# allenai/gpv-1

Hardware: AMD Instinct MI355X
Metric: images/sec/node (train step, 480x640, bs32/GPU) (higher is better)
Workload: dtype bf16; 1 GPU; GPV-1 (ResNet-50 + 6+6 DETR layers, 100 queries, RoI head, BERT-base, 3 co-attention, 3 text-decoder layers, V=10000) CocoCaptioning-only train step, dropout 0.1, AdamW; global_batch=32, image=480x640, parallelism=dp1

## Files before the change

### gpv-1_amd/csrc/misc.hip

```cpp
#include "common.h"
#include <cstdlib>
#include "../../include/gpv_hip.h"

namespace {

inline int64_t cdiv(int64_t a, int64_t b) { return (a + b - 1) / b; }
inline int grid1d(int64_t n, int per_block) {
  int64_t g = cdiv(n, per_block);
  return (int)(g > 8192 ? 8192 : (g < 1 ? 1 : g));
}

template <bool HALF> __device__ __forceinline__ float row_sum(float v) {
  if (HALF) {
#pragma unroll
    for (int o = 16; o > 0; o >>= 1) v += __shfl_xor(v, o);
    return v;
  }
  return wave_sum(v);
}

template <typename T, int NV, bool HALF>
__global__ __launch_bounds__(256) void ln_fwd_kernel(const T* __restrict__ x, const T* __restrict__ s,
                                                     const float* __restrict__ gamma, const float* __restrict__ beta,
                                                     T* __restrict__ y, float* __restrict__ mean, float* __restrict__ rstd,
// ... 339 lines not shown
}

template <typename T>
__global__ __launch_bounds__(256) void colsum8_kernel(const T* __restrict__ x, float* __restrict__ out, int rows, int cols, int64_t ld,
                                                      int ct, int rows_per_block) {
  const int cx = threadIdx.x % ct, ry = threadIdx.x / ct, rl = 256 / ct;
  const int c = ((int)blockIdx.x * ct + cx) * 8;
  if (c >= cols) return;
  const int r0 = blockIdx.y * rows_per_block, r1 = min(rows, r0 + rows_per_block);
  float s[8] = {0.f, 0.f, 0.f, 0.f, 0.f, 0.f, 0.f, 0.f};
  for (int r = r0 + ry; r < r1; r += rl) {
    float v[8];
    Ld8<T>::ld(x + (int64_t)r * ld + c, v);
#pragma unroll
    for (int e = 0; e < 8; ++e) s[e] += v[e];
  }
#pragma unroll
  for (int e = 0; e < 8; ++e) atomicAdd(&out[c + e], s[e]);
}

template <typename TS, typename TD>
__global__ void cast_kernel(const TS* __restrict__ s, TD* __restrict__ d, int64_t n) {
  for (int64_t i = blockIdx.x * (int64_t)blockDim.x + threadIdx.x; i < n; i += (int64_t)gridDim.x * blockDim.x) d[i] = (TD)(float)s[i];
}

template <typename TD>
__global__ __launch_bounds__(256) void cast_rowscale_t_kernel(const float* __restrict__ src, const float* __restrict__ scale,
                                                              TD* __restrict__ dst, TD* __restrict__ dstT, int rows, int cols) {
  __shared__ float tile[32][33];
  const int c0 = blockIdx.x * 32, r0 = blockIdx.y * 32;
  const int tx = threadIdx.x & 31, ty = threadIdx.x >> 5;
  for (int j = ty; j < 32; j += 8) {
    int r = r0 + j, c = c0 + tx;
    float v = 0.f;
    if (r < rows && c < cols) {
      v = src[(int64_t)r * cols + c] * (scale ? scale[r] : 1.f);
      if (dst) dst[(int64_t)r * cols + c] = (TD)v;
    }
    tile[j][tx] = v;
  }
  if (!dstT) return;
  __syncthreads();
  for (int j = ty; j < 32; j += 8) {
    int c = c0 + j, r = r0 + tx;
    if (r < rows && c < cols) dstT[(int64_t)c * rows + r] = (TD)tile[tx][j];
  }
}

struct TcGroup {
  int n;
  int tile_start[GPV_TC_GROUP_MAX + 1];
  gpv_tc_problem prob[GPV_TC_GROUP_MAX];
};
template <typename TD>
__global__ __launch_bounds__(256) void cast_transpose_group_kernel(const TcGroup g) {
  __shared__ float tile[64][65];
  int pi = 0;
  while (pi + 1 < g.n && (int)blockIdx.x >= g.tile_start[pi + 1]) ++pi;
  const gpv_tc_problem q = g.prob[pi];
  const int t = (int)blockIdx.x - g.tile_start[pi];
  const int tc = (q.cols + 63) >> 6;
  const int r0 = (t / tc) * 64, c0 = (t % tc) * 64;
  const int lr = threadIdx.x >> 2, seg = (threadIdx.x & 3) * 16;
  {
    const int r = r0 + lr, c = c0 + seg;
    const float* sp = q.src + (int64_t)r * q.cols + c;
    if (r < q.rows && c + 16 <= q.cols && (q.cols & 3) == 0) {
#pragma unroll
      for (int v = 0; v < 4; ++v) {
        const float4 x = *reinterpret_cast<const float4*>(sp + 4 * v);
        tile[lr][seg + 4 * v] = x.x; tile[lr][seg + 4 * v + 1] = x.y; tile[lr][seg + 4 * v + 2] = x.z; tile[lr][seg + 4 * v + 3] = x.w;
      }
    } else {
#pragma unroll
      for (int e = 0; e < 16; ++e) tile[lr][seg + e] = (r < q.rows && c + e < q.cols) ? sp[e] : 0.f;
    }
  }
  __syncthreads();
  {
    const int c = c0 + lr, r = r0 + seg;
    if (c >= q.cols) return;
    TD* dp = reinterpret_cast<TD*>(q.dstT) + (int64_t)c * q.rows + r;
    float v[16];
#pragma unroll
    for (int e = 0; e < 16; ++e) v[e] = tile[seg + e][lr];
    if (r + 16 <= q.rows && (q.rows & 7) == 0) {
      Ld8<TD>::st(dp, v);
      Ld8<TD>::st(dp + 8, v + 8);
    } else {
#pragma unroll
      for (int e = 0; e < 16; ++e)
        if (r + e < q.rows) dp[e] = (TD)v[e];
    }
  }
}

template <typename TD>
__global__ __launch_bounds__(256) void prep_conv_w_kernel(const float* __restrict__ src, const float* __restrict__ scale,
                                                          TD* __restrict__ wf, TD* __restrict__ wd, int Cout, int T, int Cin) {
  __shared__ float tile[32][33];
  const int t = blockIdx.z;
  const int ci0 = blockIdx.x * 32, co0 = blockIdx.y * 32;
  const int tx = threadIdx.x & 31, ty = threadIdx.x >> 5;
  for (int j = ty; j < 32; j += 8) {
    int co = co0 + j, ci = ci0 + tx;
    float v = 0.f;
    if (co < Cout && ci < Cin) {
      v = src[((int64_t)co * T + t) * Cin + ci] * (scale ? scale[co] : 1.f);
      if (wf) wf[((int64_t)co * T + t) * Cin + ci] = (TD)v;
    }
    tile[j][tx] = v;
  }
  if (!wd) return;
  __syncthreads();
  for (int j = ty; j < 32; j += 8) {
    int ci = ci0 + j, co = co0 + tx;
    if (co < Cout && ci < Cin) wd[((int64_t)ci * T + t) * Cout + co] = (TD)tile[tx][j];
  }
}

template <typename TT, typename TO>
__global__ void embedding_kernel(const TT* __restrict__ table, const int64_t* __restrict__ ids, TO* __restrict__ out, int64_t n_ids,
                                 int dim) {
  for (int64_t i = blockIdx.x * (int64_t)blockDim.x + threadIdx.x; i < n_ids * dim; i += (int64_t)gridDim.x * blockDim.x) {
    int64_t r = i / dim;
    int c = (int)(i - r * dim);
    out[i] = (TO)(float)table[ids[r] * dim + c];
  }
}

template <typename T>
__global__ void dropout_kernel(const T* __restrict__ x, T* __restrict__ y, int64_t n, uint32_t dthresh, float dscale, uint64_t seed,
                               const uint64_t* seed_dev) {
  seed = eff_seed(seed, seed_dev);
  for (int64_t i = blockIdx.x * (int64_t)blockDim.x + threadIdx.x; i < n; i += (int64_t)gridDim.x * blockDim.x)
    y[i] = (T)(drop_keep(seed, (uint64_t)i, dthresh) ? (float)x[i] * dscale : 0.f);
}

template <typename T>
// ... 340 lines not shown
extern "C" int gpv_colsum(const void* x, float* out, int rows, int cols, int64_t ld, int dtype, void* stream) {
  if (cols % 8 == 0 && ld % 8 == 0 && (reinterpret_cast<uintptr_t>(x) & 15) == 0) {
    const int c8 = cols / 8;
    int ct = 256;
    while (ct > 1 && ct / 2 >= c8) ct /= 2;
    const int gx = (c8 + ct - 1) / ct, rl = 256 / ct;
    int gy = (768 + gx - 1) / gx;
    if (gy > (rows + rl - 1) / rl) gy = (rows + rl - 1) / rl;
    if ((int64_t)gy * rl * cols > (1 << 17)) gy = (int)((1 << 17) / ((int64_t)rl * cols));
    if (gy < 1) gy = 1;
    const int rpb = (rows + gy - 1) / gy;
    dim3 grid(gx, (rows + rpb - 1) / rpb);
    if (dtype == GPV_BF16) hipLaunchKernelGGL((colsum8_kernel<bf16>), grid, dim3(256), 0, ST(stream), (const bf16*)x, out, rows, cols, ld, ct, rpb);
    else hipLaunchKernelGGL((colsum8_kernel<float>), grid, dim3(256), 0, ST(stream), (const float*)x, out, rows, cols, ld, ct, rpb);
    GPV_CHECK_LAUNCH();
    return 0;
  }
  int rpb = (rows + 255) / 256;
  if (rpb < 32) rpb = 32;
  dim3 grid((cols + 255) / 256, (rows + rpb - 1) / rpb);
  if (dtype == GPV_BF16) hipLaunchKernelGGL((colsum_kernel<bf16>), grid, dim3(256), 0, ST(stream), (const bf16*)x, out, rows, cols, ld, rpb);
  else hipLaunchKernelGGL((colsum_kernel<float>), grid, dim3(256), 0, ST(stream), (const float*)x, out, rows, cols, ld, rpb);
  GPV_CHECK_LAUNCH();
  return 0;
}

extern "C" int gpv_cast(const void* src, void* dst, int64_t n, int ds, int dd, void* stream) {
  dim3 g(grid1d(n, 256)), b(256);
  if (ds == GPV_F32 && dd == GPV_BF16) hipLaunchKernelGGL((cast_kernel<float, bf16>), g, b, 0, ST(stream), (const float*)src, (bf16*)dst, n);
  else if (ds == GPV_BF16 && dd == GPV_F32) hipLaunchKernelGGL((cast_kernel<bf16, float>), g, b, 0, ST(stream), (const bf16*)src, (float*)dst, n);
  else if (ds == GPV_F32 && dd == GPV_F32) hipLaunchKernelGGL((cast_kernel<float, float>), g, b, 0, ST(stream), (const float*)src, (float*)dst, n);
  else hipLaunchKernelGGL((cast_kernel<bf16, bf16>), g, b, 0, ST(stream), (const bf16*)src, (bf16*)dst, n);
  GPV_CHECK_LAUNCH();
  return 0;
}

extern "C" int gpv_cast_rowscale_t(const float* src, const float* scale, void* dst, void* dstT, int rows, int cols, int dtype_dst,
                                   void* stream) {
  dim3 grid((cols + 31) / 32, (rows + 31) / 32);
  if (dtype_dst == GPV_BF16) hipLaunchKernelGGL((cast_rowscale_t_kernel<bf16>), grid, dim3(256), 0, ST(stream), src, scale, (bf16*)dst, (bf16*)dstT, rows, cols);
  else hipLaunchKernelGGL((cast_rowscale_t_kernel<float>), grid, dim3(256), 0, ST(stream), src, scale, (float*)dst, (float*)dstT, rows, cols);
  GPV_CHECK_LAUNCH();
  return 0;
}

extern "C" int gpv_cast_transpose_group(const gpv_tc_problem* problems, int n, int dtype_dst, void* stream) {
  if (n < 0 || (n > 0 && !problems)) return (int)hipErrorInvalidValue;
  for (int i0 = 0; i0 < n; i0 += GPV_TC_GROUP_MAX) {
    TcGroup g;
    g.n = n - i0 < GPV_TC_GROUP_MAX ? n - i0 : GPV_TC_GROUP_MAX;
    int tiles = 0;
    for (int i = 0; i < g.n; ++i) {
      const gpv_tc_problem& q = problems[i0 + i];
      if (!q.src || !q.dstT || q.rows <= 0 || q.cols <= 0) return (int)hipErrorInvalidValue;
      g.prob[i] = q;
      g.tile_start[i] = tiles;
      tiles += ((q.rows + 63) / 64) * ((q.cols + 63) / 64);
    }
    g.tile_start[g.n] = tiles;
    if (dtype_dst == GPV_BF16) hipLaunchKernelGGL((cast_transpose_group_kernel<bf16>), dim3(tiles), dim3(256), 0, ST(stream), g);
    else hipLaunchKernelGGL((cast_transpose_group_kernel<float>), dim3(tiles), dim3(256), 0, ST(stream), g);
    GPV_CHECK_LAUNCH();
  }
  return 0;
}

extern "C" int gpv_prep_conv_weight(const float* src, const float* scale, void* wf, void* wd, int Cout, int T, int Cin, int dtype_dst,
                                    void* stream) {
  dim3 grid((Cin + 31) / 32, (Cout + 31) / 32, T);
  if (dtype_dst == GPV_BF16) hipLaunchKernelGGL((prep_conv_w_kernel<bf16>), grid, dim3(256), 0, ST(stream), src, scale, (bf16*)wf, (bf16*)wd, Cout, T, Cin);
  else hipLaunchKernelGGL((prep_conv_w_kernel<float>), grid, dim3(256), 0, ST(stream), src, scale, (float*)wf, (float*)wd, Cout, T, Cin);
  GPV_CHECK_LAUNCH();
  return 0;
}

extern "C" int gpv_embedding(const void* table, const int64_t* ids, void* out, int64_t n_ids, int dim, int dt, int dout, void* stream) {
  dim3 g(grid1d(n_ids * dim, 256)), b(256);
  if (dt == GPV_F32 && dout == GPV_BF16) hipLaunchKernelGGL((embedding_kernel<float, bf16>), g, b, 0, ST(stream), (const float*)table, ids, (bf16*)out, n_ids, dim);
  else if (dt == GPV_F32 && dout == GPV_F32) hipLaunchKernelGGL((embedding_kernel<float, float>), g, b, 0, ST(stream), (const float*)table, ids, (float*)out, n_ids, dim);
  else if (dt == GPV_BF16 && dout == GPV_BF16) hipLaunchKernelGGL((embedding_kernel<bf16, bf16>), g, b, 0, ST(stream), (const bf16*)table, ids, (bf16*)out, n_ids, dim);
  else return (int)hipErrorInvalidValue;
  GPV_CHECK_LAUNCH();
  return 0;
}

namespace gpvk { const uint64_t* g_seed_dev = nullptr; }
extern "C" int gpv_set_seed_device(const uint64_t* epoch) {
  gpvk::g_seed_dev = epoch;
  return 0;
}

extern "C" int gpv_dropout(const void* x, void* y, int64_t n, float p, uint64_t seed, int dtype, void* stream) {
  const uint32_t th = drop_thresh(p);
  const float sc = 1.f / (1.f - p);
  dim3 g(grid1d(n, 256)), b(256);
  if (dtype == GPV_BF16) hipLaunchKernelGGL((dropout_kernel<bf16>), g, b, 0, ST(stream), (const bf16*)x, (bf16*)y, n, th, sc, seed, gpvk::g_seed_dev);
  else hipLaunchKernelGGL((dropout_kernel<float>), g, b, 0, ST(stream), (const float*)x, (float*)y, n, th, sc, seed, gpvk::g_seed_dev);
  GPV_CHECK_LAUNCH();
  return 0;
}

extern "C" int gpv_relevance_condition(const void* x, const float* logits, const float* tokens, void* y, int rows, int dim, int dtype,
                                       void* stream) {
  dim3 g(grid1d((int64_t)rows * dim, 256)), b(256);
  if (dtype == GPV_BF16) hipLaunchKernelGGL((relevance_condition_kernel<bf16>), g, b, 0, ST(stream), (const bf16*)x, logits, tokens, (bf16*)y, rows, dim);
  else hipLaunchKernelGGL((relevance_condition_kernel<float>), g, b, 0, ST(stream), (const float*)x, logits, tokens, (float*)y, rows, dim);
  GPV_CHECK_LAUNCH();
  return 0;
}

extern "C" int gpv_act_fwd(const void* x, void* y, int64_t n, int act, int dtype, void* stream) {
  if (n % 8 || (act != GPV_ACT_RELU && act != GPV_ACT_GELU)) return (int)hipErrorInvalidValue;
// ... 52 lines not shown
```

### gpv-1_amd/hip.py

```python
import ctypes as C
import os
import threading

import torch

BF16, F32 = 0, 1
ACT_NONE, ACT_RELU, ACT_GELU = 0, 1, 2
KMAJOR, TRANS = 0, 1

_LIB = None
TUNING = os.environ.get('GPV_TUNING_LIB', '0') == '1'
_LIB_PATH = os.environ.get('GPV_HIP_LIB') or os.path.join(os.path.dirname(os.path.abspath(__file__)), 'csrc',
                                                          'libgpv_hip_tuning.so' if TUNING else 'libgpv_hip.so')


class GemmArgs(C.Structure):
    _fields_ = [('A', C.c_void_p), ('B', C.c_void_p), ('C', C.c_void_p),
                ('M', C.c_int), ('N', C.c_int), ('K', C.c_int), ('batch', C.c_int),
                ('lda', C.c_int64), ('ldb', C.c_int64), ('ldc', C.c_int64),
                ('sA', C.c_int64), ('sB', C.c_int64), ('sC', C.c_int64),
                ('layoutA', C.c_int), ('layoutB', C.c_int), ('dtype_in', C.c_int), ('dtype_out', C.c_int),
                ('alpha', C.c_float), ('rowscale', C.c_void_p), ('bias', C.c_void_p),
                ('res', C.c_void_p), ('ldr', C.c_int64), ('sR', C.c_int64),
                ('relu_mask', C.c_void_p), ('ldm', C.c_int64),
# ... 490 lines not shown
    return True


def ffn_fused_fwd(x, w1, b1, w2, b2, gamma, beta, h, y, out, mean, rstd, M, D, F, eps, drop_p=0.0, seed1=0, seed2=0, pos=None, out2=None):
    if not hasattr(lib(), 'gpv_ffn_fused_fwd'):
        return False
    ts = [t for t in (x, w1, w2, h, y, out, pos, out2) if t is not None]
    if not all(t.dtype == torch.bfloat16 and t.is_contiguous() for t in ts) or b1 is None or b2 is None:
        return False
    err = lib().gpv_ffn_fused_fwd(_p(x), _p(w1), _p(_f32(b1)), _p(w2), _p(_f32(b2)), _p(_f32(gamma)), _p(_f32(beta)), _p(h), _p(y), _p(out),
                                  _p(mean), _p(rstd), C.c_int(M), C.c_int(D), C.c_int(F), C.c_float(eps), C.c_float(drop_p), C.c_uint64(seed1), C.c_uint64(seed2),
                                  _p(pos), C.c_int(0 if pos is None else pos.numel() // D), _p(out2), _stream())
    if err == 801:
        return False
    _chk(err, 'gpv_ffn_fused_fwd')
    return True


def stem_pool(x, w, shift, y, B, Hp, Wp, CH, CW, PH, PW):
    if x.dtype != torch.bfloat16 or w.dtype != torch.bfloat16 or y.dtype != torch.bfloat16:
        raise TypeError('stem_pool: bf16 only')
    _chk(lib().gpv_stem_pool(_p(x), _p(w), _p(_f32(shift)), _p(y), B, Hp, Wp, CH, CW, PH, PW, _stream()), 'gpv_stem_pool')


def roi_weights(boxes, wgt, n_roi, H, W, ldw):
    _chk(lib().gpv_roi_weights(_p(_f32(boxes)), _p(wgt), n_roi, H, W, C.c_int64(ldw), dcode(wgt), _stream()),
         'gpv_roi_weights')


def add(a, b, y, n):
    _chk(lib().gpv_add(_p(a), _p(b), _p(y), C.c_int64(n), dcode(a), _stream()), 'gpv_add')


def add_rowbcast(a, b, y, rows_total, rows_b, cols):
    _chk(lib().gpv_add_rowbcast(_p(a), _p(b), _p(y), C.c_int64(rows_total), C.c_int64(rows_b), cols, dcode(a),
                                _stream()), 'gpv_add_rowbcast')


def colsum(x, out, rows, cols, ld):
    _chk(lib().gpv_colsum(_p(x), _p(_f32(out)), rows, cols, C.c_int64(ld), dcode(x), _stream()), 'gpv_colsum')


def cast(src, dst, n):
    _chk(lib().gpv_cast(_p(src), _p(dst), C.c_int64(n), dcode(src), dcode(dst), _stream()), 'gpv_cast')


def cast_rowscale_t(src, scale, dst, dstT, rows, cols):
    d = dst if dst is not None else dstT
    _chk(lib().gpv_cast_rowscale_t(_p(_f32(src)), _p(scale), _p(dst), _p(dstT), rows, cols, dcode(d), _stream()),
         'gpv_cast_rowscale_t')


class TCProblem(C.Structure):
    _fields_ = [('src', C.c_void_p), ('dstT', C.c_void_p), ('rows', C.c_int), ('cols', C.c_int)]


def cast_transpose_group(items):
    if not items:
        return
    arr = (TCProblem * len(items))()
    for t, (src, dstT) in zip(arr, items):
        _f32(src)
        rows, cols = src.shape
        assert src.is_contiguous() and dstT.is_contiguous() and tuple(dstT.shape) == (cols, rows)
        t.src, t.dstT, t.rows, t.cols = src.data_ptr(), dstT.data_ptr(), rows, cols
    _chk(lib().gpv_cast_transpose_group(arr, C.c_int(len(items)), C.c_int(dcode(items[0][1])), _stream()), 'gpv_cast_transpose_group')


def prep_conv_weight(src, scale, wf, wd, Cout, T, Cin):
    d = wf if wf is not None else wd
    _chk(lib().gpv_prep_conv_weight(_p(_f32(src)), _p(scale), _p(wf), _p(wd), Cout, T, Cin, dcode(d), _stream()),
         'gpv_prep_conv_weight')


def embedding(table, ids, out, n_ids, dim):
    _chk(lib().gpv_embedding(_p(table), _p(ids), _p(out), C.c_int64(n_ids), dim, dcode(table), dcode(out),
                             _stream()), 'gpv_embedding')


def dropout(x, y, n, p, seed):
    _chk(lib().gpv_dropout(_p(x), _p(y), C.c_int64(n), C.c_float(p), C.c_uint64(seed), dcode(x), _stream()),
         'gpv_dropout')


def relevance_condition(x, logits, tokens, y, rows, dim):
    _chk(lib().gpv_relevance_condition(_p(x), _p(_f32(logits)), _p(_f32(tokens)), _p(y), rows, dim, dcode(x),
                                       _stream()), 'gpv_relevance_condition')


def adamw(p, g, m, v, p_lowp, n, lr, beta1, beta2, eps, wd, bc1, bc2, gscale=None, seg_id=None, seg_live=None):
    _chk(lib().gpv_adamw(_p(p), _p(g), _p(m), _p(v), _p(p_lowp), C.c_int64(n), C.c_float(lr), C.c_float(beta1),
                         C.c_float(beta2), C.c_float(eps), C.c_float(wd), C.c_float(bc1), C.c_float(bc2),
                         _p(gscale), _p(seg_id), _p(seg_live), _stream()), 'gpv_adamw')


CLIP_PARTIALS = 1024


def clip_scale(g, max_norm, partial, gscale, pstep=None, live=None):
    n = 0 if g is None else g.numel()
    if g is not None and (not g.is_contiguous() or partial.numel() < CLIP_PARTIALS):
        raise ValueError('clip_scale: contiguous gradient range and >= CLIP_PARTIALS floats of scratch')
    for t in (pstep, live):
        if t is not None and t.dtype != torch.int32:
            raise TypeError('clip_scale: int32 step counts / liveness flags')
    _chk(lib().gpv_clip_scale(_p(_f32(g)), C.c_int64(n), C.c_float(max_norm), _p(_f32(partial)), _p(_f32(gscale)), _p(pstep), _p(live),
                              C.c_int(0 if pstep is None else pstep.numel()), _stream()), 'gpv_clip_scale')


def sumsq(x, n, out):
    _chk(lib().gpv_sumsq(_p(x), C.c_int64(n), _p(out), _stream()), 'gpv_sumsq')


def act_fwd(x, y, n, act):
    _chk(lib().gpv_act_fwd(_p(x), _p(y), C.c_int64(n), act, dcode(x), _stream()), 'gpv_act_fwd')


def argmax_rows(x, addend, out0=None, out1=None, table=None, pos_row=None, xnext=None):
    rows, V = x.shape
# ... 80 lines not shown
```

### gpv-1_amd/ops.py

```python
import math

import os
import weakref

import torch
from torch.autograd import Function

from . import hip

ACT_NONE, ACT_RELU, ACT_GELU = hip.ACT_NONE, hip.ACT_RELU, hip.ACT_GELU


class Runtime:
    def __init__(self):
        self.dtype = torch.bfloat16
        self.weights_epoch = 0
        self.static_epoch = 0
        self.seed = 0x5EED
        self.seed_explicit = False
        self._ctr = 0
        self.cache = {}
        self.backward_milestone = None
        self.split = None
        self.seed_dev = None
# ... 90 lines not shown

def _lp(p):
    N = p.shape[0]
    K = p.numel() // N
    if RT.dtype == torch.float32:
        src = p.detach().reshape(N, K)
        return src if src.is_contiguous() else src.contiguous()
    lp = getattr(p, '_gpv_lp', None)
    if lp is not None:
        if p._gpv_lp_static != RT.static_epoch:
            hip.cast(p._gpv_flat, lp, lp.numel())
            p._gpv_lp_static = RT.static_epoch
        return lp.view(N, K)
    key = ('lin', id(p), RT.dtype)
    hit = RT.cache.get(key)
    ep = RT.epoch_of(p)
    if hit is not None and hit[0] == ep:
        return hit[1]
    src = p.detach().reshape(N, K)
    if not src.is_contiguous():
        src = src.contiguous()
    w = torch.empty(N, K, device=p.device, dtype=RT.dtype)
    hip.cast(src, w, N * K)
    RT.cache[key] = (ep, w)
    return w


_T_PARAMS = {}
DX_MIRROR = os.environ.get('GPV_DX_MIRROR', '1') != '0'


def _lpT(p):
    N = p.shape[0]
    K = p.numel() // N
    key = ('linT', id(p), RT.dtype)
    hit = RT.cache.get(key)
    ep = RT.epoch_of(p)
    if hit is not None and hit[2]() is not p:
        hit = None
    if hit is not None and hit[0] == ep:
        return hit[1]
    src = getattr(p, '_gpv_flat', None)
    src = p.detach().reshape(N, K) if src is None else src.view(N, K)
    if not src.is_contiguous():
        src = src.contiguous()
    wt = hit[1] if hit is not None else torch.empty(K, N, device=p.device, dtype=RT.dtype)
    hip.cast_rowscale_t(src.float() if src.dtype != torch.float32 else src, None, None, wt, N, K)
    ref = weakref.ref(p)
    RT.cache[key] = (ep, wt, ref)
    _T_PARAMS[id(p)] = ref
    return wt


def refresh_transposed():
    items = []
    for k, r in list(_T_PARAMS.items()):
        p = r()
        hit = RT.cache.get(('linT', k, RT.dtype))
        if p is None or hit is None or hit[2]() is not p:
            _T_PARAMS.pop(k, None)
            continue
        ep = RT.epoch_of(p)
        if hit[0] == ep:
            continue
        N = p.shape[0]
        src = getattr(p, '_gpv_flat', None)
        src = p.detach().reshape(N, -1) if src is None else src.view(N, -1)
        if src.dtype != torch.float32 or not src.is_contiguous():
            _lpT(p)
            continue
        items.append((src, hit[1]))
        RT.cache[('linT', k, RT.dtype)] = (ep, hit[1], hit[2])
    hip.cast_transpose_group(items)


class W:

    def __init__(self, weight, bias=None, r0=0, r1=None):
        self.weight, self.bias = weight, bias
        self.r0 = r0
        self.r1 = weight.shape[0] if r1 is None else r1
        self.N = self.r1 - self.r0
        self.Ntot = weight.shape[0]
        self.K = weight.numel() // weight.shape[0]

    def lp(self):
        return _lp(self.weight)[self.r0:self.r1]

    def mirror_ok(self):
        return DX_MIRROR and self.weight.dim() == 2 and self.K % 8 == 0 and self.Ntot % 8 == 0 and self.r0 % 8 == 0 and self.N % 8 == 0

    def lpT(self):
        return _lpT(self.weight)[:, self.r0:self.r1]

    def dx_gemm(self, dz, dx, M, **epi):
        if self.mirror_ok():
            hip.gemm(dz, self.lpT(), dx, M, self.K, self.N, self.N, self.Ntot, self.K, **epi)
        else:
            hip.gemm(dz, self.lp(), dx, M, self.K, self.N, self.N, self.K, self.K, layoutB=hip.TRANS, **epi)

    def bias_f32(self):
        return None if self.bias is None else self.bias.detach()[self.r0:self.r1]

    def wgrad(self):
        g = ensure_grad(self.weight)
        return g.reshape(self.Ntot, self.K)[self.r0:self.r1]

    def bgrad(self):
        return ensure_grad(self.bias)[self.r0:self.r1]


def _split_k(out_rows, out_cols, red):
    tiles = ((out_rows + 63) // 64) * ((out_cols + 63) // 64)
    kt = (red + 31) // 32
    return max(1, min(-(-768 // max(tiles, 1)), 8, kt // 16))


def _c(x):
    return x if x.is_contiguous() else x.contiguous()


def _as_compute(x):
    return x if x.dtype == RT.dtype else x.to(RT.dtype)


class GradChain:
# ... 255 lines not shown
    with torch.cuda.stream(st):
        cap = torch.cuda.is_current_stream_capturing()
    if cap:
        waiter.wait_stream(st)


def branch_for(x):
    if not (Branch.ENABLED and torch.is_tensor(x) and x.is_cuda):
        return None
    if torch.cuda.is_current_stream_capturing():
        st = RT.branch_stream
        return Branch(x.device, st) if st is not None else None
    st = Branch._streams.get(x.device)
    if st is None:
        st = Branch._streams[x.device] = torch.cuda.Stream(device=x.device)
    return Branch(x.device, st)


_MULTI = {}


def _multi_key(ws):
    return ('multi', tuple((id(w.weight), w.r0, w.r1) for w in ws), RT.dtype)


def _multi_build(ws, old=None):
    o = old if old is not None else (None, None, None)
    wcat = torch.cat([w.lp() for w in ws], 0, out=o[0])
    bcat = torch.cat([w.bias_f32() for w in ws], 0, out=o[1]) if ws[0].bias is not None else None
    wT = torch.cat([w.lpT() for w in ws], 1, out=o[2]) if all(w.mirror_ok() for w in ws) else None
    return wcat, bcat, wT


def _multi_get(ws):
    key = _multi_key(ws)
    ep = max(RT.epoch_of(w.weight) for w in ws)
    hit = RT.cache.get(key)
    if hit is not None and hit[0] == ep and all(r() is w.weight for r, w in zip(hit[4], ws)):
        return hit[1:4]
    same = hit is not None and all(r() is w.weight for r, w in zip(hit[4], ws))
    built = _multi_build(ws, hit[1:4] if same else None)
    RT.cache[key] = (ep,) + built + (tuple(weakref.ref(w.weight) for w in ws),)
    _MULTI[key] = tuple(ws)
    return built


def refresh_multi():
    for key, ws in list(_MULTI.items()):
        hit = RT.cache.get(key)
        if hit is None or key[2] != RT.dtype or any(r() is not w.weight for r, w in zip(hit[4], ws)):
            _MULTI.pop(key, None)
            continue
        ep = max(RT.epoch_of(w.weight) for w in ws)
        RT.cache[key] = (ep,) + _multi_build(ws, hit[1:4]) + (hit[4],)


class MultiLinearFn(Function):

    @staticmethod
    def forward(ctx, x, ws, sink=None, chain=None):
        ctx.sink = sink
        ctx.chain = chain.join() if (chain is not None and ctx.needs_input_grad[0]) else None
        K, N, n = ws[0].K, ws[0].N, len(ws)
        x2 = _c(_as_compute(x)).reshape(-1, K)
        M = x2.shape[0]
        if RT.multi_wait is not None:
            RT.multi_wait()
        wcat, bcat, _ = _multi_get(ws)
        y = torch.empty(M, n * N, device=x.device, dtype=RT.dtype)
        hip.gemm(x2, wcat, y, M, n * N, K, K, K, n * N, bias=bcat)
        ctx.ws, ctx.xshape = ws, x.shape
        ctx.save_for_backward(x2)
        return y

    @staticmethod
    def backward(ctx, dy):
        ws = ctx.ws
        (x2,) = ctx.saved_tensors
        K, N, n = ws[0].K, ws[0].N, len(ws)
        M = x2.shape[0]
        dz = _c(_as_compute(dy)).reshape(M, n * N)
        if ctx.sink is not None:
            ctx.sink.release()
        for i, w in enumerate(ws):
            need_b = w.bias is not None and w.bias.requires_grad
            if w.weight.requires_grad:
                wgrad_linear(dz[:, i * N:(i + 1) * N], x2, w.wgrad(), w.bgrad() if need_b else None, N, K, M, _split_k(N, K, M), lda=n * N)
            elif need_b:
                hip.colsum(dz[:, i * N:(i + 1) * N], w.bgrad(), M, N, n * N)
        dx = None
        if ctx.needs_input_grad[0]:
            dx = torch.empty(M, K, device=dz.device, dtype=RT.dtype)
            wcat, _, wT = _multi_get(ws)
            ch = ctx.chain
            epi = {'res': ch.acc.reshape(M, K), 'ldr': K} if (ch is not None and ch.acc is not None) else {}
            if wT is not None:
                hip.gemm(dz, wT, dx, M, K, n * N, n * N, n * N, K, **epi)
            else:
                hip.gemm(dz, wcat, dx, M, K, n * N, n * N, K, K, layoutB=hip.TRANS, **epi)
            dx = dx.reshape(ctx.xshape)
            if ch is not None:
                dx = ch.done(dx)
        return dx, None, None, None


def multi_linear(x, ws, sink=None, chain=None):
# ... 612 lines not shown
```

### gpv-1_amd/train.py

```python
import collections
import gc
import os
import time

import torch
import torch.distributed as dist

from . import hip
from .ops import RT

GROUPS = ('detr_backbone', 'detr_head', 'bert', 'others')


def param_group_of(name):
    if 'detr.backbone' in name:
        return 'detr_backbone'
    if 'detr' in name:
        return 'detr_head'
    if 'bert.' in name:
        return 'bert'
    return 'others'


NEVER_GRAD = ('bert.', 'vision_token', 'lang_token', 'q_dense1', 'q_dense2', 'pos_enc', 'vocab_embed', 'embedding_layer',
# ... 98 lines not shown
            torch.cuda.current_stream(dev).wait_stream(self.wside)
            _ops.Branch.join_captured(dev)
            _ops.foreign_capturing((self.side, self.wside, self.bside), 'F2 end')
            self.f2.capture_end()
            self._open = None
            _ops.still_capturing((('side', self.side), ('wside', self.wside), ('bside', self.bside)), 'after F2')
        except BaseException:
            self._abort_open()
            raise
        finally:
            RT.split = None
            RT.branch_stream = None
            RT.multi_wait = None
            self.chains, _ops.GradChain._live = _ops.GradChain._live, live_before
        self.fwd_touched = trainer.touched.clone()
        trainer._captures += 1
        trainer.touched |= saved

    def _abort_open(self):
        g, self._open = self._open, None
        if g is not None:
            try:
                g.capture_end()
            except Exception:
                pass
        for st in (self.side, self.wside, self.bside):
            if st is not None:
                try:
                    st.synchronize()
                except Exception:
                    pass

    def backbone_forward(self, body, x, train=True, hw=None):
        self.keep = [] if train else None
        c5 = body.forward_nhwc(x, self.keep, hw)
        if self.bert_mode == 1:
            torch.cuda.current_stream(x.device).wait_stream(self.side)
        self._prep_forked = False
        self.f1.capture_end()
        self._open = None
        from . import ops as _ops2
        _ops2.still_capturing((('side', self.side), ('wside', self.wside), ('bside', self.bside)), 'after F1')
        self.f2.capture_begin(pool=self.pool, capture_error_mode=CAPTURE_MODE)
        self._open = self.f2
        if self.bert_mode == 2:
            cur = torch.cuda.current_stream(x.device)
            self.side.wait_stream(cur)
            with torch.cuda.stream(self.side), torch.no_grad():
                self._q_enc, _ = self.tr.model.bert((self.s_ids, self.s_attn))
        from . import ops
        cur = torch.cuda.current_stream(x.device)
        self.wside.wait_stream(cur)
        with torch.cuda.stream(self.wside):
            ops.refresh_transposed()
            ops.refresh_multi()
            multi_ready = torch.cuda.Event()
            multi_ready.record(self.wside)
            if self.zero_in_graph:
                self.tr.G.zero_()
        waited = set()

        def multi_wait():
            cur = torch.cuda.current_stream(x.device)
            if cur.cuda_stream not in waited:
                cur.wait_event(multi_ready)
                waited.add(cur.cuda_stream)
        RT.multi_wait = multi_wait
        self.c5 = c5
        self.c5_leaf = c5.detach().requires_grad_(bool(train))
        self.body = body
        return self.c5_leaf

    def _bert_join(self):
        torch.cuda.current_stream(self.s_img.device).wait_stream(self.side)
        return self._q_enc

    def prep_fork(self, body):
        if os.environ.get('GPV_PREP_BRANCH', '1') == '0':
            return
        cur = torch.cuda.current_stream(self.s_img.device)
        self.wside.wait_stream(cur)
        with torch.cuda.stream(self.wside):
            body.prep_weights()
            self._prep_done = torch.cuda.Event()
            self._prep_done.record(self.wside)
        self._prep_forked = True

    def prep_join(self):
        if getattr(self, '_prep_forked', False):
            torch.cuda.current_stream(self.s_img.device).wait_event(self._prep_done)

    def stale(self):
        return self.epochs != (RT.static_epoch, RT.dtype)

    def __del__(self):
        try:
            from .ops import retire
            streams = [getattr(self, n, None) for n in ('side', 'wside', 'bside')]
            graphs = [getattr(self, n, None) for n in ('f1', 'f2')] + list(getattr(self, 'variants', {}).values())
            self.f1 = self.f2 = None
            if hasattr(self, 'variants'):
                self.variants.clear()
            self.keep = None
            retire(graphs, streams)
        except Exception:
            pass

    def forward(self, images, queries, tok, lang_extra=None, leaves=True):
        from . import backbone as bbm
        self.s_img.copy_(images.tensors, non_blocking=True)
        self.s_mask.copy_(images.mask, non_blocking=True)
        self.s_ids.copy_(queries[0], non_blocking=True)
# ... 799 lines not shown
```

### include/gpv_hip.h

```cpp
#ifndef GPV_HIP_H
#define GPV_HIP_H
#include <stdint.h>
#ifdef __cplusplus
extern "C" {
#endif

#define GPV_BF16 0
#define GPV_F32 1

#define GPV_ACT_NONE 0
#define GPV_ACT_RELU 1
#define GPV_ACT_GELU 2

#define GPV_KMAJOR 0
#define GPV_TRANS 1

int gpv_abi_version(void);
int gpv_build_id(char* buf, int cap);

#define GPV_TT_GROUP_MAX 48
typedef struct {
  const void* A; const void* B; float* C; float* a_rowsum;
  int M, N, K;
  int lda, ldb, ldc;
// ... 132 lines not shown
  float drop_p; uint64_t seed;
  float* lse;
  int dtype;
  const void* dout; int64_t do_bs, do_rs;
  void* dq; void* dk; void* dv;
} gpv_attn_args;
int gpv_attention_fwd(const gpv_attn_args* a, void* stream);
int gpv_attention_bwd(const gpv_attn_args* a, void* stream);
int gpv_attention_qkv_fwd(const gpv_attn_args* a, const void* xp, const void* x, int64_t x_bs, int64_t x_rs, const void* w,
                          const float* bias, void* stream);

int gpv_layernorm_fwd(const void* x, const void* s, const float* gamma, const float* beta, void* y,
                      float* mean, float* rstd, int rows, int cols, float eps, float drop_p,
                      uint64_t seed, int dtype, void* stream);
int gpv_layernorm_bwd(const void* dy, const void* x, const void* s, const float* gamma,
                      const float* mean, const float* rstd, void* dx, void* ds, float* dgamma,
                      float* dbeta, int rows, int cols, float drop_p, uint64_t seed, int dtype,
                      void* stream);
int gpv_layernorm_pos_fwd(const void* x, const void* s, const float* gamma, const float* beta, void* y, float* mean, float* rstd,
                          int rows, int cols, float eps, float drop_p, uint64_t seed, const void* pos, int pos_rows, void* y2,
                          int dtype, void* stream);
int gpv_layernorm_bwd2(const void* dy, const void* dy2, const void* x, const void* s, const float* gamma, const float* mean,
                       const float* rstd, void* dx, void* ds, float* dgamma, float* dbeta, int rows, int cols, float drop_p,
                       uint64_t seed, int dtype, void* stream);

int gpv_linear_layernorm_fwd(const void* a, const void* w, const float* bias, const void* x, const float* gamma, const float* beta,
                             void* s, void* y, float* mean, float* rstd, int rows, int K, int N, float eps, float drop_p, uint64_t seed,
                             const void* pos, int pos_rows, void* y2, void* stream);
typedef struct gpv_fold_problem {
  const float* partials;
  float* out0;
  float* out1;
  int nblk, cols;
} gpv_fold_problem;
int gpv_layernorm_bwd_blocks(int rows, int cols);
int gpv_layernorm_bwd3(const void* dy, const void* dy2, const void* x, const void* s, const float* gamma, const float* mean,
                       const float* rstd, void* dx, void* ds, float* dgamma, float* dbeta, float* partials, int rows, int cols,
                       float drop_p, uint64_t seed, int dtype, void* stream);
int gpv_colsum_fold_group(const gpv_fold_problem* problems, int n, void* stream);

int gpv_softmax_ce(const void* logits, int64_t ld, const int64_t* target, float* loss, void* dlogits,
                   const float* gscale, int rows, int V, int dtype, void* stream);

int gpv_roi_weights(const float* boxes, void* wgt, int n_roi, int H, int W, int64_t ldw, int dtype,
                    void* stream);

int gpv_add(const void* a, const void* b, void* y, int64_t n, int dtype, void* stream);
int gpv_add_rowbcast(const void* a, const void* b, void* y, int64_t rows_total, int64_t rows_b,
                     int cols, int dtype, void* stream);
int gpv_colsum(const void* x, float* out, int rows, int cols, int64_t ld, int dtype, void* stream);
int gpv_cast(const void* src, void* dst, int64_t n, int dtype_src, int dtype_dst, void* stream);
int gpv_cast_rowscale_t(const float* src, const float* scale, void* dst, void* dstT, int rows, int cols,
                        int dtype_dst, void* stream);
#define GPV_TC_GROUP_MAX 128
typedef struct { const float* src; void* dstT; int rows, cols; } gpv_tc_problem;
int gpv_cast_transpose_group(const gpv_tc_problem* problems, int n, int dtype_dst, void* stream);
int gpv_prep_conv_weight(const float* src, const float* scale, void* wf, void* wd, int Cout, int T,
                         int Cin, int dtype_dst, void* stream);
int gpv_embedding(const void* table, const int64_t* ids, void* out, int64_t n_ids, int dim, int dtype_table,
                  int dtype_out, void* stream);
int gpv_argmax_rows(const void* x, int64_t ld, const float* addend, int rows, int V, int dtype,
                    int64_t* out0, int64_t stride0, int64_t* out1, int64_t stride1, void* stream);
int gpv_argmax_rows_embed(const void* x, int64_t ld, const float* addend, int rows, int V, int dtype,
                          int64_t* out0, int64_t stride0, int64_t* out1, int64_t stride1,
                          const void* table, int64_t ldt, const void* pos_row, void* xnext, int D, void* stream);
int gpv_ln_linear_rows(const void* x, const void* s, const float* gamma, const float* beta, float eps, void* xn,
                       const void* W, int64_t ldw, const float* bias, void* y, int64_t ldy,
                       int rows, int N, int K, int act, int dtype, const float* s_partial, int s_parts, const float* s_bias,
                       void* stream);
int gpv_attention_row_proj(const void* q, int64_t q_bs, const void* k, int64_t k_bs, int64_t k_rs, const void* v, int64_t v_bs,
                           int64_t v_rs, const void* Wo, int64_t ldw, float* partial, int B, int H, int Sk, int dh, float scale,
                           int dtype, void* stream);
int gpv_act_fwd(const void* x, void* y, int64_t n, int act, int dtype, void* stream);
int gpv_act_bwd(const void* dy, const void* ref, void* dx, int64_t n, int act, float alpha, int dtype, void* stream);
int gpv_dropout(const void* x, void* y, int64_t n, float p, uint64_t seed, int dtype, void* stream);
int gpv_set_seed_device(const uint64_t* epoch);
int gpv_relevance_condition(const void* x, const float* logits, const float* tokens, void* y, int rows,
                            int dim, int dtype, void* stream);

int gpv_adamw(float* p, const float* g, float* m, float* v, void* p_lowp, int64_t n, float lr, float beta1,
              float beta2, float eps, float wd, float bc1, float bc2, const float* gscale,
              const uint16_t* seg_id, const int32_t* seg_live, void* stream);
int gpv_sumsq(const float* x, int64_t n, float* out , void* stream);
#define GPV_CLIP_PARTIALS 1024
int gpv_clip_scale(const float* g, int64_t n, float max_norm, float* partial, float* gscale, int32_t* pstep, const int32_t* live,
                   int nparam, void* stream);

#ifdef __cplusplus
}
#endif
#endif
```

Measured before the change: 2135 images/sec.

## Fuse weight refresh, multi-weight concat and grad zeroing into one grouped kernel

```diff
diff --git a/gpv-1_amd/csrc/misc.hip b/gpv-1_amd/csrc/misc.hip
--- a/gpv-1_amd/csrc/misc.hip
+++ b/gpv-1_amd/csrc/misc.hip
@@ -415,6 +415,43 @@
   int tile_start[GPV_TC_GROUP_MAX + 1];
   gpv_tc_problem prob[GPV_TC_GROUP_MAX];
 };
+static_assert(sizeof(TcGroup) <= 4096, "TcGroup travels as a kernel argument");
+
+__device__ __forceinline__ bool tc_al16(const void* p) { return (reinterpret_cast<uintptr_t>(p) & 15) == 0; }
+
+template <typename TS, typename TO, bool LOAD>
+__device__ __forceinline__ void tc_copy16(const TS* sp, TO* dp, int nv, bool svec, bool dvec) {
+  float v[16];
+  if (!LOAD) {
+#pragma unroll
+    for (int e = 0; e < 16; ++e) v[e] = 0.f;
+  } else if (svec && nv == 16) {
+    Ld8<TS>::ld(sp, v);
+    Ld8<TS>::ld(sp + 8, v + 8);
+  } else {
+#pragma unroll
+    for (int e = 0; e < 16; ++e) v[e] = e < nv ? (float)sp[e] : 0.f;
+  }
+  if (dvec && nv == 16) {
+    Ld8<TO>::st(dp, v);
+    Ld8<TO>::st(dp + 8, v + 8);
+  } else {
+#pragma unroll
+    for (int e = 0; e < 16; ++e)
+      if (e < nv) dp[e] = (TO)v[e];
+  }
+}
+
+template <typename TS, typename TO, bool LOAD>
+__device__ __forceinline__ void tc_copy_tile(const gpv_tc_problem& q, int r0, int c0, int lds, int ldd) {
+  const int r = r0 + (threadIdx.x >> 2), c = c0 + (threadIdx.x & 3) * 16;
+  if (r >= q.rows || c >= q.cols) return;
+  const int nv = q.cols - c < 16 ? q.cols - c : 16;
+  const bool svec = LOAD && tc_al16(q.src) && (lds & 7) == 0, dvec = tc_al16(q.dstT) && (ldd & 7) == 0;
+  tc_copy16<TS, TO, LOAD>(reinterpret_cast<const TS*>(q.src) + (int64_t)r * lds + c, reinterpret_cast<TO*>(q.dstT) + (int64_t)r * ldd + c,
+                          nv, svec, dvec);
+}
+
 template <typename TD>
 __global__ __launch_bounds__(256) void cast_transpose_group_kernel(const TcGroup g) {
   __shared__ float tile[64][65];
@@ -424,11 +461,21 @@
   const int t = (int)blockIdx.x - g.tile_start[pi];
   const int tc = (q.cols + 63) >> 6;
   const int r0 = (t / tc) * 64, c0 = (t % tc) * 64;
+  const int lds = q.lds ? q.lds : q.cols;
+  if (q.mode != GPV_TC_TRANSPOSE) {
+    const int ldd = q.ldd ? q.ldd : q.cols;
+    if (q.mode == GPV_TC_COPY_CAST) tc_copy_tile<float, TD, true>(q, r0, c0, lds, ldd);
+    else if (q.mode == GPV_TC_COPY) tc_copy_tile<TD, TD, true>(q, r0, c0, lds, ldd);
+    else if (q.mode == GPV_TC_COPY_F32) tc_copy_tile<float, float, true>(q, r0, c0, lds, ldd);
+    else tc_copy_tile<float, float, false>(q, r0, c0, lds, ldd);
+    return;
+  }
+  const int ldd = q.ldd ? q.ldd : q.rows;
   const int lr = threadIdx.x >> 2, seg = (threadIdx.x & 3) * 16;
   {
     const int r = r0 + lr, c = c0 + seg;
-    const float* sp = q.src + (int64_t)r * q.cols + c;
-    if (r < q.rows && c + 16 <= q.cols && (q.cols & 3) == 0) {
+    const float* sp = reinterpret_cast<const float*>(q.src) + (int64_t)r * lds + c;
+    if (r < q.rows && c + 16 <= q.cols && (lds & 3) == 0 && tc_al16(q.src)) {
 #pragma unroll
       for (int v = 0; v < 4; ++v) {
         const float4 x = *reinterpret_cast<const float4*>(sp + 4 * v);
@@ -443,11 +490,11 @@
   {
     const int c = c0 + lr, r = r0 + seg;
     if (c >= q.cols) return;
-    TD* dp = reinterpret_cast<TD*>(q.dstT) + (int64_t)c * q.rows + r;
+    TD* dp = reinterpret_cast<TD*>(q.dstT) + (int64_t)c * ldd + r;
     float v[16];
 #pragma unroll
     for (int e = 0; e < 16; ++e) v[e] = tile[seg + e][lr];
-    if (r + 16 <= q.rows && (q.rows & 7) == 0) {
+    if (r + 16 <= q.rows && (ldd & 7) == 0 && tc_al16(q.dstT)) {
       Ld8<TD>::st(dp, v);
       Ld8<TD>::st(dp + 8, v + 8);
     } else {
@@ -894,12 +941,18 @@
     int tiles = 0;
     for (int i = 0; i < g.n; ++i) {
       const gpv_tc_problem& q = problems[i0 + i];
-      if (!q.src || !q.dstT || q.rows <= 0 || q.cols <= 0) return (int)hipErrorInvalidValue;
+      if (q.rows < 0 || q.cols < 0 || q.mode < GPV_TC_TRANSPOSE || q.mode > GPV_TC_ZERO_F32 || q.lds < 0 || q.ldd < 0) return (int)hipErrorInvalidValue;
+      const bool empty = q.rows == 0 || q.cols == 0;
+      if (!empty) {
+        if (!q.dstT || (!q.src && q.mode != GPV_TC_ZERO_F32)) return (int)hipErrorInvalidValue;
+        if ((q.lds && q.lds < q.cols) || (q.ldd && q.ldd < (q.mode == GPV_TC_TRANSPOSE ? q.rows : q.cols))) return (int)hipErrorInvalidValue;
+      }
       g.prob[i] = q;
       g.tile_start[i] = tiles;
-      tiles += ((q.rows + 63) / 64) * ((q.cols + 63) / 64);
+      if (!empty) tiles += ((q.rows + 63) / 64) * ((q.cols + 63) / 64);
     }
     g.tile_start[g.n] = tiles;
+    if (tiles == 0) continue;
     if (dtype_dst == GPV_BF16) hipLaunchKernelGGL((cast_transpose_group_kernel<bf16>), dim3(tiles), dim3(256), 0, ST(stream), g);
     else hipLaunchKernelGGL((cast_transpose_group_kernel<float>), dim3(tiles), dim3(256), 0, ST(stream), g);
     GPV_CHECK_LAUNCH();
diff --git a/gpv-1_amd/hip.py b/gpv-1_amd/hip.py
--- a/gpv-1_amd/hip.py
+++ b/gpv-1_amd/hip.py
@@ -566,19 +566,39 @@
 
 
 class TCProblem(C.Structure):
-    _fields_ = [('src', C.c_void_p), ('dstT', C.c_void_p), ('rows', C.c_int), ('cols', C.c_int)]
+    _fields_ = [('src', C.c_void_p), ('dstT', C.c_void_p), ('rows', C.c_int), ('cols', C.c_int), ('lds', C.c_int), ('ldd', C.c_int), ('mode', C.c_int)]
+
+
+TC_TRANSPOSE, TC_COPY_CAST, TC_COPY, TC_COPY_F32, TC_ZERO_F32 = range(5)
 
 
 def cast_transpose_group(items):
     if not items:
         return
+    for src, dstT in items:
+        assert src.is_contiguous() and dstT.is_contiguous()
+    publish_group([(TC_TRANSPOSE, src, dstT) for src, dstT in items], items[0][1].dtype)
+
+
+def publish_group(items, dtype):
+    if not items:
+        return
     arr = (TCProblem * len(items))()
-    for t, (src, dstT) in zip(arr, items):
-        _f32(src)
-        rows, cols = src.shape
-        assert src.is_contiguous() and dstT.is_contiguous() and tuple(dstT.shape) == (cols, rows)
-        t.src, t.dstT, t.rows, t.cols = src.data_ptr(), dstT.data_ptr(), rows, cols
-    _chk(lib().gpv_cast_transpose_group(arr, C.c_int(len(items)), C.c_int(dcode(items[0][1])), _stream()), 'gpv_cast_transpose_group')
+    for t, (mode, src, dst) in zip(arr, items):
+        sd, dd = {TC_TRANSPOSE: (torch.float32, dtype), TC_COPY_CAST: (torch.float32, dtype), TC_COPY: (dtype, dtype),
+                  TC_COPY_F32: (torch.float32, torch.float32), TC_ZERO_F32: (None, torch.float32)}[mode]
+        rows, cols = (dst.shape if src is None else src.shape)
+        want = (cols, rows) if mode == TC_TRANSPOSE else (rows, cols)
+        if dst.dim() != 2 or tuple(dst.shape) != want or dst.dtype != dd or (dst.numel() and dst.stride(1) != 1 and dst.shape[1] > 1):
+            raise ValueError('publish_group: destination %s %s for a mode %d source of %s' % (tuple(dst.shape), dst.dtype, mode, (rows, cols)))
+        if src is not None and (src.dim() != 2 or src.dtype != sd or (src.numel() and src.stride(1) != 1 and src.shape[1] > 1)):
+            raise ValueError('publish_group: source %s %s in mode %d' % (tuple(src.shape), src.dtype, mode))
+        t.src = _p(src).value if (src is not None and src.numel()) else None
+        t.dstT = _p(dst).value if dst.numel() else None
+        t.rows, t.cols, t.mode = rows, cols, mode
+        t.lds = src.stride(0) if (src is not None and rows > 1) else 0
+        t.ldd = dst.stride(0) if dst.shape[0] > 1 else 0
+    _chk(lib().gpv_cast_transpose_group(arr, C.c_int(len(items)), C.c_int(dcode(torch.empty(0, dtype=dtype))), _stream()), 'gpv_cast_transpose_group')
 
 
 def prep_conv_weight(src, scale, wf, wd, Cout, T, Cin):
diff --git a/gpv-1_amd/ops.py b/gpv-1_amd/ops.py
--- a/gpv-1_amd/ops.py
+++ b/gpv-1_amd/ops.py
@@ -166,7 +166,7 @@
     return wt
 
 
-def refresh_transposed():
+def _stale_transposed():
     items = []
     for k, r in list(_T_PARAMS.items()):
         p = r()
@@ -185,7 +185,11 @@
             continue
         items.append((src, hit[1]))
         RT.cache[('linT', k, RT.dtype)] = (ep, hit[1], hit[2])
-    hip.cast_transpose_group(items)
+    return items
+
+
+def refresh_transposed():
+    hip.cast_transpose_group(_stale_transposed())
 
 
 class W:
@@ -547,6 +551,67 @@
             _MULTI.pop(key, None)
             continue
         ep = max(RT.epoch_of(w.weight) for w in ws)
+        RT.cache[key] = (ep,) + _multi_build(ws, hit[1:4]) + (hit[4],)
+
+
+def _multi_items(ws, built):
+    wcat, bcat, wT = built
+    if (bcat is None) != (ws[0].bias is None) or (wT is None) != (not all(w.mirror_ok() for w in ws)):
+        return None
+    items, r = [], 0
+    for w in ws:
+        items.append((hip.TC_COPY, w.lp(), wcat[r:r + w.N]))
+        if bcat is not None:
+            b = w.bias_f32()
+            if b.dtype != torch.float32 or not b.is_contiguous():
+                return None
+            items.append((hip.TC_COPY_F32, b.view(1, -1), bcat[r:r + w.N].view(1, -1)))
+        if wT is not None:
+            src = getattr(w.weight, '_gpv_flat', None)
+            src = w.weight.detach().reshape(w.Ntot, w.K) if src is None else src.view(w.Ntot, w.K)
+            if src.dtype != torch.float32 or not src.is_contiguous():
+                return None
+            items.append((hip.TC_TRANSPOSE, src[w.r0:w.r1], wT[:, r:r + w.N]))
+        r += w.N
+    return items
+
+
+GLUE_FUSED = os.environ.get('GPV_GLUE_FUSED', '1') != '0'
+
+
+def refresh_derived(zero=None):
+    if not GLUE_FUSED:
+        refresh_transposed()
+        refresh_multi()
+        if zero is not None:
+            zero.zero_()
+        return
+    items = [(hip.TC_TRANSPOSE, src, dstT) for src, dstT in _stale_transposed()]
+    late = []
+    for key, ws in list(_MULTI.items()):
+        hit = RT.cache.get(key)
+        if hit is None or key[2] != RT.dtype or any(r() is not w.weight for r, w in zip(hit[4], ws)):
+            _MULTI.pop(key, None)
+            continue
+        ep = max(RT.epoch_of(w.weight) for w in ws)
+        site = _multi_items(ws, hit[1:4])
+        if site is None:
+            late.append((key, ws, ep, hit))
+            continue
+        items += site
+        RT.cache[key] = (ep,) + tuple(hit[1:4]) + (hit[4],)
+    if zero is not None:
+        if zero.dtype != torch.float32 or not zero.is_contiguous():
+            zero.zero_()
+        else:
+            flat = zero.view(-1)
+            n = flat.numel() // 64 * 64
+            if n:
+                items.append((hip.TC_ZERO_F32, None, flat[:n].view(-1, 64)))
+            if flat.numel() - n:
+                items.append((hip.TC_ZERO_F32, None, flat[n:].view(1, -1)))
+    hip.publish_group(items, RT.dtype)
+    for key, ws, ep, hit in late:
         RT.cache[key] = (ep,) + _multi_build(ws, hit[1:4]) + (hit[4],)
 
 
diff --git a/gpv-1_amd/train.py b/gpv-1_amd/train.py
--- a/gpv-1_amd/train.py
+++ b/gpv-1_amd/train.py
@@ -174,12 +174,9 @@
         cur = torch.cuda.current_stream(x.device)
         self.wside.wait_stream(cur)
         with torch.cuda.stream(self.wside):
-            ops.refresh_transposed()
-            ops.refresh_multi()
+            ops.refresh_derived(self.tr.G if self.zero_in_graph else None)
             multi_ready = torch.cuda.Event()
             multi_ready.record(self.wside)
-            if self.zero_in_graph:
-                self.tr.G.zero_()
         waited = set()
 
         def multi_wait():
diff --git a/include/gpv_hip.h b/include/gpv_hip.h
--- a/include/gpv_hip.h
+++ b/include/gpv_hip.h
@@ -208,8 +208,13 @@
 int gpv_cast(const void* src, void* dst, int64_t n, int dtype_src, int dtype_dst, void* stream);
 int gpv_cast_rowscale_t(const float* src, const float* scale, void* dst, void* dstT, int rows, int cols,
                         int dtype_dst, void* stream);
-#define GPV_TC_GROUP_MAX 128
-typedef struct { const float* src; void* dstT; int rows, cols; } gpv_tc_problem;
+#define GPV_TC_GROUP_MAX 80
+#define GPV_TC_TRANSPOSE 0
+#define GPV_TC_COPY_CAST 1
+#define GPV_TC_COPY 2
+#define GPV_TC_COPY_F32 3
+#define GPV_TC_ZERO_F32 4
+typedef struct { const void* src; void* dstT; int rows, cols; int lds, ldd; int mode; } gpv_tc_problem;
 int gpv_cast_transpose_group(const gpv_tc_problem* problems, int n, int dtype_dst, void* stream);
 int gpv_prep_conv_weight(const float* src, const float* scale, void* wf, void* wd, int Cout, int T,
                          int Cin, int dtype_dst, void* stream);
```

Result: slower. 2097 images/sec (-1.8%).
